# SciML/NeuralPDE.jl

Hardware: AMD Instinct MI355X
Metric: collocation-point residual+grad evals/sec, 2D Poisson 4x64 MLP (higher is better)
Workload: dtype f32, hidden-layer forward / dA / dW GEMMs as 3-piece bf16 split products (6 bf16 MFMAs per product block, fp32 accumulation; 24 mantissa bits rebuilt; the five small piece products on an accumulator of their own: zero-mean, a third of the rms error of an fp32-MFMA fmaf chain per GEMM output, tools/m

## Files before the change

### neuralpde.jl_amd/csrc/pinn_kernels2.hpp

```cpp
#pragma once
#include "pinn_kernels.hpp"

#if defined(PINN_STAMP) && !defined(PINN_EMU)
#define STAMP_MEMBERS unsigned st_acc[24]; unsigned long long st_last;
#define STAMP_INIT(ac) { for (int i_ = 0; i_ < 24; ++i_) (ac).st_acc[i_] = 0; (ac).st_last = __builtin_amdgcn_s_memtime(); }
#define STAMP(i) { const unsigned long long st_now = __builtin_amdgcn_s_memtime(); ac.st_acc[i] += (unsigned)(st_now - ac.st_last); ac.st_last = st_now; }
#define STAMP_EXTRA 128
#else
#define STAMP_MEMBERS
#define STAMP_INIT(ac)
#define STAMP(i)
#define STAMP_EXTRA 0
#endif

#ifndef PINN_F2_REC_LDS
#define PINN_F2_REC_LDS 1
#endif
#ifndef PINN_F2_SWP
#define PINN_F2_SWP 7
#endif
#ifndef PINN_PROBE
#define PINN_PROBE 0
#endif
#ifndef PINN_F2_ADJ_IL
#define PINN_F2_ADJ_IL 1
#endif
#ifndef PINN_F2_TR_FWDIMG
#define PINN_F2_TR_FWDIMG 1
#endif
#ifndef PINN_F2_SPLIT_ACC2
#define PINN_F2_SPLIT_ACC2 1
#endif
#ifndef PINN_F2_WACC_PRELOAD
#define PINN_F2_WACC_PRELOAD 2
#endif
#ifndef PINN_F2_MODES
#define PINN_F2_MODES 3
#endif

namespace pk {

constexpr int GEMM_FP32 = 0, GEMM_SPLIT = 1;
constexpr int F2_WAVES128 = 8;
constexpr int F2_NW8_MAXNG = 6;
constexpr int F2_GEMM_AHEAD = 2;
// ... 146 lines not shown
                ac.wLbar[t][r] = gload_masked(slab + S::O_WL, n, c0i);
            }
        if (w == 0) {
            const vbool l0 = veq(lane, 0);
            ac.bLbar = gload_masked(slab + S::O_BL, lane & vint(0), l0);
            PINN_UNROLL for (int j = 0; j < MAX_PARAMS; ++j) ac.pbar[j] = gload_masked(slab + S::O_P, vint(j) + (lane & vint(0)), l0);
        }
    }
}

template <class S, int MODE, int ACTK>
DEV void wave_tiles2(const GroupArgs& ga, int blk, int nblocks, int w, float* lds, Acc2<typename S::Shape>& ac,
                     int term_lo, int term_hi, int tile_lo, int tile_hi) {
    constexpr int HP = S::HP, MT = S::MT, MTW = S::MTW, NHH = S::NHH, LH = S::LH, D = S::D, C = S::C, PG = S::PG, NG = S::NG;
    constexpr int NFIRST = S::NFIRST;
    using J = typename S::J;
    constexpr bool BWD = (MODE == MODE_FUSED || MODE == MODE_GRADIN || MODE == MODE_GRADREC);
    constexpr bool SUMS = (MODE == MODE_FUSED || MODE == MODE_LOSS);
    constexpr bool TAPE_ONLY = (MODE == MODE_RESID || MODE == MODE_LOSS);
    constexpr bool RECOUT = (MODE == MODE_FWDREC), RECIN = (MODE == MODE_GRADREC);
    constexpr bool IS_FWD = (MODE == MODE_FWD || MODE == MODE_FWDREC), IS_GRADIN = (MODE == MODE_GRADIN || MODE == MODE_GRADREC);
    constexpr bool WPRE = (MT * MTW * 4 <= 16);
    constexpr bool TR_OVL = S::BFX_TR && WPRE && !S::CHUNKED;
    const int wave = blk * S::NW + w;
    const vint lane = lane_id();
    const vint g = lane >> 4;
    const vint c = lane & vint(15);
    const vbool g0 = veq(g, 0);
    const vint sw = S::BFX_TR ? (((g << 4) + (c ^ ((g >> 1) << 2))) << 1) : (lane << 2);
    vint trb[2];
    PINN_UNROLL for (int jh = 0; jh < 2; ++jh) {
        const vint gg = c & vint(3), pc = ((g & vint(1)) << 3) + vint(4 * jh) + (c >> 2);
        trb[jh] = (((gg << 4) + (pc ^ ((gg >> 1) << 2))) << 1);
    }
    vint trbq[2];
    PINN_UNROLL for (int jh = 0; jh < 2; ++jh) trbq[jh] = trb[jh] + (g >> 1) * vint(S::KB * 3 * 256);
    const vbool klo = vlt(g, 2);
    const float* P = ga.packed;
    constexpr int act = ACTK;
    static_assert(ACTK != ACT_MIXED, "per-layer activation kinds are compiled for family 1 (small nets) only");
    constexpr int ACLS = act_class(ACTK);
    constexpr bool RECZ = act_records_z(ACLS);
    const ubuf PB = ub_make(P, S::PACKED);
    const ubuf SB = ub_make(ga.scratch + (size_t)blk * (ga.scr_stride ? ga.scr_stride : S::SCR), S::SCR);
    float* X0 = lds;
    float* X1 = lds + S::OFF_X1;
// ... 6 lines not shown
    float* slab = ga.slabs + (size_t)blk * S::SLAB;
    auto& wbar = ac.wbar;
    auto& bbar = ac.bbar;
    auto& w1bar = ac.w1bar;
    auto& wLbar = ac.wLbar;
    vfloat& bLbar = ac.bLbar;
    auto& pbar = ac.pbar;
    vdacc& lsum = ac.lsum;
    int& cur_term = ac.cur_term;

    auto ld_wf = [&](int hl, int t, int mi) -> vfloat4 {
        return ub_load4(PB, S::OFF_WPK + ((hl * MT + w * MTW + t) * MT + mi) * 256, lane << 2);
    };
    auto ld_wt = [&](int hl, int t, int mo) -> vfloat4 {
        return ub_load4(PB, S::OFF_WTPK + ((hl * MT + w * MTW + t) * MT + mo) * 256, lane << 2);
    };
    auto ld_bias = [&](int layer, int t) -> vfloat4 { return ub_load4(PB, S::off_b(layer) + 16 * (w * MTW + t), g << 2); };

    vfloat4 wL[MTW];
    PINN_UNROLL for (int t = 0; t < MTW; ++t) wL[t] = ub_load4(PB, S::OFF_WL + 16 * (w * MTW + t), g << 2);
    const vbf8 wb_probe = ((PINN_PROBE & 8) && S::BFIMG) ? ub_load_bf8(PB, S::OFF_WB, lane << 2) : vbf8{};
    const float bL = P[S::OFF_BL];

    wave_prio(1);
    const int first = tile_lo + (((blk - tile_lo) % nblocks) + nblocks) % nblocks;
    for (int tix = first; tix < tile_hi; tix += nblocks) {
        STAMP(15)
        int k = term_lo;
        for (int j = term_lo + 1; j < term_hi; ++j)
            if (tix >= ga.terms[j].tile0) k = j;
        if (k != cur_term) {
            if (cur_term >= 0 && SUMS)
                ga.losspart[(size_t)wave * ga.nterms_total + ga.terms[cur_term].term_id] = wave_sum_dd(lsum, g0);
            lsum = vdacc_zero();
            cur_term = k;
        }
        const TermDev& T = ga.terms[k];
        const int pbase = (tix - T.tile0) * S::TP;
        const ubuf RB = ub_make((RECOUT || RECIN) ? ga.rec + (size_t)tix * S::REC : ga.scratch, S::REC);

        vfloat x[PG][D];
        vbool valid[PG];
        PINN_UNROLL for (int pg = 0; pg < PG; ++pg) {
            vint p = vint(pbase + 16 * pg) + c;
            valid[pg] = vlt(p, T.N);
            PINN_UNROLL for (int i = 0; i < D; ++i) x[pg][i] = gload_masked(T.pts, p * T.dt + vint(T.imap[i]), valid[pg]);
        }

        vfloat4 Rlast[NG][MTW];
        auto act_forward = [&](vfloat4 (&Z)[NG][MTW], int layer) {
            PINN_UNROLL for (int pg = 0; pg < PG; ++pg)
                PINN_UNROLL for (int t = 0; t < MTW; ++t) {
                    vfloat4 av;
                    av = act_value4<ACLS>(act, Z[pg * C][t]);
                    if (!RECZ) Z[pg * C][t] = av;
                    if (RECOUT && layer > 0)
                        PINN_UNROLL for (int ch = 0; ch < C; ++ch)
                            ub_store4(RB, (((layer - 1) * NG + pg * C + ch) * MT + w * MTW + t) * 256, lane << 2, Z[pg * C + ch][t]);
                    if (BWD) {
                        if (layer == LH - 1) {
                            PINN_UNROLL for (int ch = 0; ch < C; ++ch) Rlast[pg * C + ch][t] = Z[pg * C + ch][t];
                        } else if (layer > 0) {
                            PINN_UNROLL for (int ch = 0; ch < C; ++ch) {
                                if (rec_in_lds(layer, pg * C + ch)) lds_store4(RL, rl_off(layer, pg * C + ch, t), Z[pg * C + ch][t]);
                                else ub_store4(SB, (((layer - 1) * NG + pg * C + ch) * MT + w * MTW + t) * 256, lane << 2, Z[pg * C + ch][t]);
                            }
                        }
                    }
                    if ((RECOUT && layer > 0) || (BWD && layer > 0 && layer != LH - 1 && !rec_in_lds(layer, pg * C + C - 1))) {
// ... 110 lines not shown
                    PINN_UNROLL for (int sp = 0; sp < 3; ++sp) bb[(i + 1) % NB][sp] = ld_bfrag(X, (q2 * S::KB + kb2) * 3 + sp);
                }
                sched_fence();
                if (i + 1 < NGRP) lds_wait<3 * RD>(); else lds_wait<0>();
                PINN_UNROLL for (int t = 0; t < MTW; ++t) {
                    if (acc == 1) mfma_split2(wfr[kb][t], bb[i % NB], Cc[q][t], Cs[q][t]);
                    else Cc[q][t] = mfma_split(wfr[kb][t], bb[i % NB], Cc[q][t]);
                }
                chain_fence();
            }
            if (acc == 1)
                PINN_UNROLL for (int q = 0; q < NG; ++q)
                    PINN_UNROLL for (int t = 0; t < MTW; ++t)
                        PINN_UNROLL for (int e = 0; e < 4; ++e) Cc[q][t][e] += Cs[q][t][e];
        };
#ifndef PINN_F2_ACC_2PASS_ALL
#define PINN_F2_ACC_2PASS_ALL 0
#endif
        constexpr bool ACC_2PASS = PINN_F2_ACC_2PASS_ALL || (HP >= 128 && NG >= 5);
        auto acc_mode = [&](int bit) -> int { return (PINN_F2_SPLIT_ACC2 & bit) ? (ACC_2PASS ? 2 : 1) : 0; };

        vfloat4 A[NG][MTW];
        vfloat U[PG][C];
        constexpr int SRC_PRE = 2;
        vfloat srcv[SRC_PRE];
        PINN_UNROLL for (int j = 0; j < SRC_PRE; ++j) srcv[j] = vfloat(0.f);
        vbool valid_w = valid[0];
        PINN_UNROLL for (int pg = 1; pg < PG; ++pg) if (w == pg) valid_w = valid[pg];
        if (!RECIN) {
            PINN_UNROLL for (int t = 0; t < MTW; ++t) {
                const int n0 = 16 * (w * MTW + t);
                vfloat4 b1 = ub_load4(PB, S::off_b(0) + n0, g << 2);
                vfloat4 w1[D];
                PINN_UNROLL for (int i = 0; i < D; ++i) w1[i] = ub_load4(PB, S::OFF_W1 + i * HP + n0, g << 2);
                PINN_UNROLL for (int pg = 0; pg < PG; ++pg) {
                    vfloat4 z = b1;
                    PINN_UNROLL for (int i = 0; i < D; ++i)
                        PINN_UNROLL for (int r = 0; r < 4; ++r) z[r] = vfma(w1[i][r], x[pg][i], z[r]);
                    A[pg * C][t] = z;
                    PINN_UNROLL for (int kf = 0; kf < NFIRST; ++kf) A[pg * C + 1 + kf][t] = w1[S::first_axis(kf)];
                    PINN_UNROLL for (int ch = 1 + NFIRST; ch < C; ++ch) A[pg * C + ch][t] = vzero4();
                }
            }
            act_forward(A, 0);
            STAMP(0)
            PINN_UNROLL for (int hl = 0; hl < NHH; ++hl) {
                float* Xin = (hl & 1) ? X1 : X0;
// ... 52 lines not shown
                            PINN_UNROLL for (int t = 0; t < MTW; ++t)
                                PINN_UNROLL for (int e = 0; e < 4; ++e) A[q][t][e] += As[q][t][e];
                    if (WPRE && F2_GEMM_AHEAD > 0) sched_gemm_prefetch<S::KB * NG, MTW * 6, F2_GEMM_AHEAD, S::BFX_TR ? 6 : 3>();
                }
                PINN_UNROLL for (int mi = 0; mi < (S::BFX ? 0 : MT); ++mi) {
                    if (!WPRE)
                        PINN_UNROLL for (int t = 0; t < MTW; ++t)
                            wf[0][t] = ld_wf(hl, t, mi);
                    vfloat4 b4[NG];
                    PINN_UNROLL for (int q = 0; q < NG; ++q) b4[q] = lds_load4(Xin, vint(((q * MT + mi) * 64) * 4) + (lane << 2));
                    PINN_UNROLL for (int q = 0; q < NG; ++q)
                        PINN_UNROLL for (int t = 0; t < MTW; ++t)
                            PINN_UNROLL for (int rr = 0; rr < 4; ++rr) A[q][t] = mfma16(wf[WPRE ? mi : 0][t][rr], b4[q][rr], A[q][t]);
                }
                if (!S::BFX && WPRE && F2_GEMM_AHEAD > 0) sched_gemm_prefetch<MT * NG, MTW * 4, F2_GEMM_AHEAD>();
                wave_prio(1);
                STAMP(2)
                act_forward(A, hl + 1);
                STAMP(3)
            }
            if (MODE == MODE_FUSED || TAPE_ONLY)
                if (w < PG)
                    PINN_UNROLL for (int j = 0; j < SRC_PRE; ++j)
                        if (j < T.nsrc) srcv[j] = gload_masked(T.src, vint(j * T.N + pbase + 16 * w) + c, valid_w);
            {
                PINN_UNROLL for (int q = 0; q < NG; ++q) {
                    vfloat s = vfloat(0.f);
                    PINN_UNROLL for (int t = 0; t < MTW; ++t)
                        PINN_UNROLL for (int r = 0; r < 4; ++r) s = vfma(wL[t][r], A[q][t][r], s);
                    s = xrow_allsum(s);
                    lds_store(UP, vint((w * NG + q) * 16) + c, s);
                }
                wg_barrier();
            }
            PINN_UNROLL for (int pg = 0; pg < PG; ++pg)
                PINN_UNROLL for (int ch = 0; ch < C; ++ch) {
                    vfloat s = vfloat(0.f);
                    PINN_UNROLL for (int ws = 0; ws < S::NW; ++ws) s = s + lds_load(UP, vint((ws * NG + pg * C + ch) * 16) + c);
                    U[pg][ch] = (ch == 0) ? s + vfloat(bL) : s;
                }
        } else {
            PINN_UNROLL for (int pg = 0; pg < PG; ++pg)
                PINN_UNROLL for (int ch = 0; ch < C; ++ch) U[pg][ch] = vfloat(0.f);
            if (LH == 1) {
                PINN_UNROLL for (int t = 0; t < MTW; ++t) {
                    const int n0 = 16 * (w * MTW + t);
                    vfloat4 b1 = ub_load4(PB, S::off_b(0) + n0, g << 2);
// ... 11 lines not shown
                }
            } else {
                PINN_UNROLL for (int q = 0; q < NG; ++q)
                    PINN_UNROLL for (int t = 0; t < MTW; ++t)
                        Rlast[q][t] = ub_load4(RB, (((LH - 2) * NG + q) * MT + w * MTW + t) * 256, lane << 2);
            }
            PINN_UNROLL for (int pg = 0; pg < PG; ++pg)
                PINN_UNROLL for (int t = 0; t < MTW; ++t)
                    PINN_UNROLL for (int r = 0; r < 4; ++r) {
                        vfloat zz[C], dd[ND];
                        PINN_UNROLL for (int k2 = 0; k2 < C; ++k2) zz[k2] = Rlast[pg * C + k2][t][r];
                        act_derivs_n<J::NORD - 1, ACLS>(act, zz[0], dd);
                        jet_forward<J>(zz, dd);
                        A[pg * C][t][r] = act_from_record<ACLS>(Rlast[pg * C][t][r]);
                        PINN_UNROLL for (int k2 = 1; k2 < C; ++k2) A[pg * C + k2][t][r] = zz[k2];
                    }
        }
        STAMP(4)
        if (IS_FWD) {
            if (w == 0)
                PINN_UNROLL for (int pg = 0; pg < PG; ++pg) {
                    vint p = vint(pbase + 16 * pg) + c;
                    PINN_UNROLL for (int ch = 0; ch < C; ++ch)
                        gstore_masked(T.out, vint(ch * T.N) + p, U[pg][ch], vand(valid[pg], g0));
                }
            wg_barrier();
            continue;
        }

        constexpr bool SPRE = (NG * MTW * 4 <= F2_SPRE_MAX);
        vfloat4 Snext[SPRE ? NG : 1][SPRE ? MTW : 1];
        auto load_record = [&](int hl) {
            PINN_UNROLL for (int q = 0; q < NG; ++q)
                PINN_UNROLL for (int t = 0; t < MTW; ++t)
                    Snext[q][t] = (!RECIN && rec_in_lds(hl, q)) ? lds_load4(RL, rl_off(hl, q, t))
                                                             : ub_load4(RECIN ? RB : SB, (((hl - 1) * NG + q) * MT + w * MTW + t) * 256, lane << 2);
            sched_fence();
        };
        vfloat ubar[PG][C];
        if (IS_GRADIN) {
            PINN_UNROLL for (int pg = 0; pg < PG; ++pg) {
                vint p = vint(pbase + 16 * pg) + c;
                PINN_UNROLL for (int ch = 0; ch < C; ++ch) ubar[pg][ch] = gload_masked(T.in, vint(ch * T.N) + p, valid[pg]);
            }
            if (SPRE && NHH - 1 >= 1) load_record(NHH - 1);
        } else {
            float* UB = UP + S::NW * NG * 16;
            if (w < PG) {
                wave_prio(3);
                vfloat xin[D], Uin[C];
                vbool vin = valid[0];
                PINN_UNROLL for (int i = 0; i < D; ++i) xin[i] = x[0][i];
                PINN_UNROLL for (int ch = 0; ch < C; ++ch) Uin[ch] = U[0][ch];
                PINN_UNROLL for (int pg = 1; pg < PG; ++pg)
                    if (w == pg) {
                        vin = valid[pg];
                        PINN_UNROLL for (int i = 0; i < D; ++i) xin[i] = x[pg][i];
                        PINN_UNROLL for (int ch = 0; ch < C; ++ch) Uin[ch] = U[pg][ch];
                    }
                if (T.linear && C <= LIN_MAX_C) {
                    vfloat r = vfloat(T.lin_k);
                    PINN_UNROLL for (int ch = 0; ch < C; ++ch) r = vfma(vfloat(T.lin_a[ch < LIN_MAX_C ? ch : 0]), Uin[ch], r);
                    PINN_UNROLL for (int j = 0; j < LIN_MAX_SRC; ++j)
                        if (j < T.nsrc) {
                            vfloat sv;
                            if (j < SRC_PRE) { PINN_UNROLL for (int jj = 0; jj < SRC_PRE; ++jj) if (jj == j) sv = srcv[jj]; }
                            else sv = gload_masked(T.src, vint(j * T.N + pbase + 16 * w) + c, vin);
                            r = vfma(vfloat(T.lin_b[j]), sv, r);
                        }
                    if (MODE == MODE_RESID) {
                        vint p = vint(pbase + 16 * w) + c;
                        gstore_masked(T.out, p, r, vand(vin, g0));
                    } else {
                        vfloat sw = vfloat(1.0f);
                        if (T.pw) sw = gload_masked(T.pw, vint(pbase + 16 * w) + c, vin);
                        vfloat rm = vselect(vin, r * sw, vfloat(0.f));
                        lsum = vdacc_fma(rm, vselect(g0, rm, vfloat(0.f)), lsum);
                        if (MODE != MODE_LOSS) {
                            vfloat rbar = rm * vfloat(T.scale) * sw;
                            PINN_UNROLL for (int ch = 0; ch < C; ++ch)
                                lds_store(UB, vint((w * C + ch) * 16) + c, vselect(vin, rbar * vfloat(T.lin_a[ch < LIN_MAX_C ? ch : 0]), vfloat(0.f)));
                            if (T.src_bar)
                                PINN_UNROLL for (int j = 0; j < LIN_MAX_SRC; ++j)
                                    if (j < T.nsrc) gstore_masked(T.src_bar, vint(j * T.N + pbase + 16 * w) + c, rbar * vfloat(T.lin_b[j]), vand(vin, g0));
                        }
                    }
                } else {
                    const int NP = ga.nparams;
                    const int DT = T.dt;
                    const int R0 = DT + NP + C + T.nsrc;
                    const rp::Instr* prog = ga.prog + T.prog_off;
                    vtape tv;
                    tape_zero(tv);
                    if (!T.hetero) {
                        PINN_UNROLL for (int i = 0; i < D; ++i) tape_set(tv, i, xin[i]);
                    } else {
                        for (int j = 0; j < DT; ++j) tape_set(tv, j, gload_masked(T.pts, (vint(pbase + 16 * w) + c) * DT + vint(j), vin));
                    }
                    for (int j = 0; j < NP; ++j) tape_set(tv, DT + j, vfloat(ga.params[j]));
                    PINN_UNROLL for (int ch = 0; ch < C; ++ch) tape_set(tv, DT + NP + ch, Uin[ch]);
                    for (int j = 0; j < T.nsrc; ++j) {
                        vfloat sv;
                        if (j < SRC_PRE) { PINN_UNROLL for (int jj = 0; jj < SRC_PRE; ++jj) if (jj == j) sv = srcv[jj]; }
                        else sv = gload_masked(T.src, vint(j * T.N + pbase + 16 * w) + c, vin);
                        tape_set(tv, DT + NP + C + j, sv);
                    }
                    for (int q = 0; q < T.nops; ++q) {
                        const rp::Instr ins = rp::fetch_uniform(prog, q);
                        const vfloat va = tape_get(tv, ins.a), vb = tape_get(tv, ins.b);
                        vfloat vo;
                        if (rp::is_bilinear(ins.code)) vo = rp::apply_bilinear<vfloat>(ins, va, vb);
                        else vo = rp::apply<vfloat>(ins.code, va, vb, ins.imm);
                        tape_set(tv, R0 + q, vo);
                    }
                    vfloat r = tape_get(tv, T.out_row);
                    if (MODE == MODE_RESID) {
                        vint p = vint(pbase + 16 * w) + c;
                        gstore_masked(T.out, p, r, vand(vin, g0));
                    } else {
                        vfloat sw = vfloat(1.0f);
                        if (T.pw) sw = gload_masked(T.pw, vint(pbase + 16 * w) + c, vin);
                        vfloat rm = vselect(vin, r * sw, vfloat(0.f));
                        lsum = vdacc_fma(rm, vselect(g0, rm, vfloat(0.f)), lsum);
                        if (MODE != MODE_LOSS) {
                        vfloat rbar = rm * vfloat(T.scale) * sw;
                        vtape ta;
                        tape_zero(ta);
                        tape_set(ta, T.out_row, vfloat(1.0f));
                        for (int q = T.nops - 1; q >= 0; --q) {
                            const rp::Instr ins = rp::fetch_uniform(prog, q);
                            const vfloat va = tape_get(tv, ins.a), vb = tape_get(tv, ins.b), gq = tape_get(ta, R0 + q);
                            vfloat da, db;
                            if (rp::is_bilinear(ins.code)) rp::adjoint_bilinear<vfloat>(ins, va, vb, gq, da, db);
                            else rp::adjoint<vfloat>(ins.code, va, vb, tape_get(tv, R0 + q), ins.imm, gq, da, db);
                            tape_set(ta, ins.a, tape_get(ta, ins.a) + da);
                            tape_set(ta, ins.b, tape_get(ta, ins.b) + db);
                        }
                        PINN_UNROLL for (int ch = 0; ch < C; ++ch)
                            lds_store(UB, vint((w * C + ch) * 16) + c, vselect(vin, rbar * tape_get(ta, DT + NP + ch), vfloat(0.f)));
                        if (T.src_bar)
                            for (int j = 0; j < T.nsrc; ++j)
                                gstore_masked(T.src_bar, vint(j * T.N + pbase + 16 * w) + c, rbar * tape_get(ta, DT + NP + C + j), vand(vin, g0));
                        for (int j = 0; j < ga.nparams_estim; ++j) {
                            vfloat pj = vselect(vand(g0, vin), rbar * tape_get(ta, DT + j), vfloat(0.f));
                            PINN_UNROLL for (int jj = 0; jj < MAX_PARAMS; ++jj) if (jj == j) pbar[jj] += pj;
                        }
                        }
                    }
                }
                }
            wave_prio(1);
            if (!TAPE_ONLY) {
                if (SPRE && NHH - 1 >= 1) load_record(NHH - 1);
                wg_barrier();
                PINN_UNROLL for (int pg = 0; pg < PG; ++pg)
                    PINN_UNROLL for (int ch = 0; ch < C; ++ch) ubar[pg][ch] = lds_load(UB, vint((pg * C + ch) * 16) + c);
            }
        }
        if (TAPE_ONLY) { wg_barrier(); continue; }
        STAMP(5)

        constexpr bool FWD_IMG = S::BFX_TR && !RECIN && NHH >= 1 && PINN_F2_TR_FWDIMG;
        float* XA = (S::BFX_TR && ((NHH - 1) & 1) == 0) ? X0 : X1;
        float* XZ = (S::BFX_TR && ((NHH - 1) & 1) == 0) ? X1 : X0;
        auto ajet = [&](const vfloat4 (&Sr)[NG][MTW], int pg, int ch, int t) -> vfloat4 {
            vfloat4 out;
            PINN_UNROLL for (int r = 0; r < 4; ++r) {
                vfloat zz[C], dd[ND];
                PINN_UNROLL for (int k = 0; k < C; ++k) zz[k] = Sr[pg * C + k][t][r];
                if (ch > 0) {
                    act_derivs_n<J::NORD - 1, ACLS>(act, zz[0], dd);
                    jet_forward<J>(zz, dd);
                }
                out[r] = (ch == 0) ? act_from_record<ACLS>(zz[0]) : zz[ch];
            }
            return out;
        };
        auto act_adjoint = [&](vfloat4 (&G)[NG][MTW], const vfloat4 (&Sr)[NG][MTW]) {
            PINN_UNROLL for (int pg = 0; pg < PG; ++pg)
                PINN_UNROLL for (int t = 0; t < MTW; ++t)
                    PINN_UNROLL for (int r = 0; r < 4; ++r) {
                        vfloat gg[C], ss[C], dd[ND];
// ... 170 lines not shown
            };
            vfloat4 wt[WPRE ? MT : 1][MTW];
            vbf8 wtb[S::BFX ? S::KB : 1][S::BFX ? MTW : 1][3];
            if (S::BFX) {
                PINN_UNROLL for (int kb = 0; kb < S::KB; ++kb)
                    PINN_UNROLL for (int t = 0; t < MTW; ++t)
                        PINN_UNROLL for (int sp = 0; sp < 3; ++sp)
                            wtb[kb][t][sp] = (PINN_PROBE & 8) ? wb_probe : ub_load_bf8(PB, S::OFF_WTB + (((hl * MT + w * MTW + t) * S::KB + kb) * 3 + sp) * 256, lane << 2);
                sched_fence();
            } else if (WPRE) {
                PINN_UNROLL for (int mo = 0; mo < MT; ++mo)
                    PINN_UNROLL for (int t = 0; t < MTW; ++t)
                        wt[mo][t] = ld_wt(hl, t, mo);
                sched_fence();
            }
            vfloat4 Gn[NG][MTW];
            PINN_UNROLL for (int q = 0; q < NG; ++q)
                PINN_UNROLL for (int t = 0; t < MTW; ++t) Gn[q][t] = vzero4();
            constexpr bool OVL = WPRE && !S::CHUNKED;
            if (OVL) {
                STAMP(7)
                wg_barrier();
                STAMP(8)
                if (SPRE && hl - 1 >= 1) load_record(hl - 1);
                wave_prio(0);
                if (S::BFX_TR && (PINN_F2_SWP & 2)) gemm_swp(XZ, wtb, Gn, acc_mode(2));
                PINN_UNROLL for (int q = 0; q < ((S::BFX_TR && (PINN_F2_SWP & 2)) ? 0 : NG); ++q) {
                    if (S::BFX) {
                        constexpr bool ACC2 = (PINN_F2_SPLIT_ACC2 & 2) != 0;
                        vfloat4 Gs[MTW];
                        PINN_UNROLL for (int t = 0; t < MTW; ++t) Gs[t] = vzero4();
                        PINN_UNROLL for (int kb = 0; kb < S::KB; ++kb) {
                            vbf8 bb[3];
                            PINN_UNROLL for (int sp = 0; sp < 3; ++sp) bb[sp] = ld_bfrag(XZ, (q * S::KB + kb) * 3 + sp);
                            PINN_UNROLL for (int t = 0; t < MTW; ++t) {
                                if (ACC2) mfma_split2(wtb[kb][t], bb, Gn[q][t], Gs[t]);
                                else Gn[q][t] = mfma_split(wtb[kb][t], bb, Gn[q][t]);
                            }
                        }
                        if (ACC2)
                            PINN_UNROLL for (int t = 0; t < MTW; ++t)
                                PINN_UNROLL for (int e = 0; e < 4; ++e) Gn[q][t][e] += Gs[t][e];
                    } else {
                        PINN_UNROLL for (int mo = 0; mo < MT; ++mo) {
                            vfloat4 b4 = lds_load4(X0, vint(((q * MT + mo) * 64) * 4) + (lane << 2));
                            PINN_UNROLL for (int t = 0; t < MTW; ++t)
// ... 125 lines not shown
            }
            STAMP(10)
            wg_barrier();
            STAMP(11)
            if (!ADJ_IL) {
                PINN_UNROLL for (int q = 0; q < NG; ++q)
                    PINN_UNROLL for (int t = 0; t < MTW; ++t) G[q][t] = Gn[q][t];
                act_adjoint(G, Sr);
            }
            STAMP(12)
        }
        PINN_UNROLL for (int pg = 0; pg < PG; ++pg)
            PINN_UNROLL for (int t = 0; t < MTW; ++t)
                PINN_UNROLL for (int r = 0; r < 4; ++r) {
                    const vfloat gz = G[pg * C][t][r];
                    bbar[0][t][r] += gz;
                    PINN_UNROLL for (int i = 0; i < D; ++i) w1bar[i][t][r] = vfma(gz, x[pg][i], w1bar[i][t][r]);
                    PINN_UNROLL for (int kf = 0; kf < NFIRST; ++kf)
                        PINN_UNROLL for (int i = 0; i < D; ++i)
                            if (i == S::first_axis(kf)) w1bar[i][t][r] += G[pg * C + 1 + kf][t][r];
                }
        if (NHH == 0) wg_barrier();
        STAMP(13)
    }
}

template <class S, int PG = S::PG >
DEV void acc2_store(Acc2<typename S::Shape>& ac, const GroupArgs& ga, int blk, int w, float* lds) {
    constexpr int HP = S::HP, MT = S::MT, MTW = S::MTW, NHH = S::NHH, LH = S::LH, D = S::D, NG = S::NG;
    const vint lane = lane_id();
    const vint g = lane >> 4;
    const vint c = lane & vint(15);
    float* slab = ga.slabs + (size_t)blk * S::SLAB;
    float* UP = lds + S::OFF_UP;
    if (S::WBAR_REG)
        PINN_UNROLL for (int hl = 0; hl < NHH; ++hl)
            PINN_UNROLL for (int t = 0; t < MTW; ++t)
                PINN_UNROLL for (int ti = 0; ti < MT; ++ti)
                    gstore4(slab + S::O_WBAR, vint((((hl * MT + w * MTW + t) * MT + ti) * 64) * 4) + (lane << 2), ac.wbar[hl][t][ti]);
    const vbool c0 = veq(c, 0);
    auto reduce_cols = [&](vfloat v) -> vfloat {
        v = row_allsum16(v);
        return v;
    };
    PINN_UNROLL for (int t = 0; t < MTW; ++t)
        PINN_UNROLL for (int r = 0; r < 4; ++r) {
// ... 12 lines not shown
    if (w == 0) {
        float s = (float)wave_sum_d(ac.bLbar, all);
        gstore_masked(slab + S::O_BL, vint(0), vfloat(s), veq(lane, 0));
        PINN_UNROLL for (int j = 0; j < MAX_PARAMS; ++j) {
            vfloat sp = vfloat((float)wave_sum_d(ac.pbar[j], all));
            PINN_UNROLL for (int ws = 1; ws < PG; ++ws) sp = sp + lds_load(UBp, vint(ws * MAX_PARAMS + j) + (lane & vint(0)));
            gstore_masked(slab + S::O_P, vint(j), sp, veq(lane, 0));
        }
    }
#if defined(PINN_STAMP) && !defined(PINN_EMU)
    STAMP(14)
    if ((threadIdx.x & 63) == 0)
        for (int i = 0; i < 24; ++i) reinterpret_cast<unsigned*>(slab + S::SLAB - 128)[w * 24 + i] = ac.st_acc[i];
#endif
}

template <class S, int MODE, int ACTK>
DEV void wave_main2(const GroupArgs& ga, int blk, int nblocks, int w, float* lds) {
    constexpr bool BWD = (MODE == MODE_FUSED || MODE == MODE_GRADIN || MODE == MODE_GRADREC);
    constexpr bool SUMS = (MODE == MODE_FUSED || MODE == MODE_LOSS);
    const int wave = blk * S::NW + w;
    Acc2<typename S::Shape> ac;
    acc2_init<S>(ac, ga, blk, w, BWD);
    if (SUMS)
        for (int j = 0; j < ga.nterms; ++j) ga.losspart[(size_t)wave * ga.nterms_total + ga.terms[j].term_id] = 0.0;
    wave_tiles2<S, MODE, ACTK>(ga, blk, nblocks, w, lds, ac, 0, ga.nterms, 0, ga.ntiles);
    if (SUMS && ac.cur_term >= 0)
        ga.losspart[(size_t)wave * ga.nterms_total + ga.terms[ac.cur_term].term_id] = wave_sum_dd(ac.lsum, veq(lane_id() >> 4, 0));
    if (!BWD) return;
    acc2_store<S>(ac, ga, blk, w, lds);
}

template <class S0, class S1, int ACTK, int MODE = MODE_FUSED>
DEV void wave_main2m(const GroupArgs& ga, int blk, int nblocks, int w, float* lds) {
    static_assert(same_type<typename S0::Shape, typename S1::Shape>::value, "merged launches need members of one network shape and neuron split");
    static_assert(S0::SLAB == S1::SLAB && S0::PACKED == S1::PACKED, "merged launches share the slab and the packed weight image");
    static_assert(S0::DW_NATURAL == S1::DW_NATURAL && S0::BFX_TR == S1::BFX_TR, "merged launches: one order of the dW tiles in the slab, one exchange-image layout");
    static_assert(MODE == MODE_FUSED || MODE == MODE_LOSS, "merged launches: the fused evaluation and the loss-only evaluation");
    const int wave = blk * S0::NW + w;
    Acc2<typename S0::Shape> ac;
    acc2_init<S0>(ac, ga, blk, w, MODE == MODE_FUSED);
    for (int j = 0; j < ga.nterms; ++j) ga.losspart[(size_t)wave * ga.nterms_total + ga.terms[j].term_id] = 0.0;
    wave_tiles2<S0, MODE, ACTK>(ga, blk, nblocks, w, lds, ac, 0, ga.sub_terms0, 0, ga.sub_tiles0);
    wg_barrier();
    wave_tiles2<S1, MODE, ACTK>(ga, blk, nblocks, w, lds, ac, ga.sub_terms0, ga.nterms, ga.sub_tiles0, ga.ntiles);
    if (ac.cur_term >= 0)
        ga.losspart[(size_t)wave * ga.nterms_total + ga.terms[ac.cur_term].term_id] = wave_sum_dd(ac.lsum, veq(lane_id() >> 4, 0));
    if (MODE != MODE_FUSED) return;
    wg_barrier();
    acc2_store<S0, (S0::PG > S1::PG ? S0::PG : S1::PG)>(ac, ga, blk, w, lds);
}

}
```

### neuralpde.jl_amd/csrc/vec.hpp

```cpp
#pragma once
#ifndef __HIPCC_RTC__
#include <cmath>
#include <cstdint>
#include <cstring>
#include <type_traits>
#endif

#ifdef PINN_EMU
#define DEV inline
#define HD inline
#define PINN_UNROLL
namespace wv {
constexpr int W = 64;
struct vbool { bool v[W]; };
struct vint {
    int v[W];
    vint() {}
    vint(int s) { for (int l = 0; l < W; ++l) v[l] = s; }
};
struct vfloat {
    float v[W];
    vfloat() {}
    vfloat(float s) { for (int l = 0; l < W; ++l) v[l] = s; }
};
// ... 54 lines not shown
#undef VFN1
inline vfloat vpow(const vfloat& a, const vfloat& b) { vfloat r; for (int l = 0; l < W; ++l) r.v[l] = std::pow(a.v[l], b.v[l]); return r; }
inline vfloat vmax(const vfloat& a, const vfloat& b) { vfloat r; for (int l = 0; l < W; ++l) r.v[l] = a.v[l] > b.v[l] ? a.v[l] : b.v[l]; return r; }
inline vfloat vmin(const vfloat& a, const vfloat& b) { vfloat r; for (int l = 0; l < W; ++l) r.v[l] = a.v[l] < b.v[l] ? a.v[l] : b.v[l]; return r; }
inline vbool vlt(const vint& a, int b) { vbool r; for (int l = 0; l < W; ++l) r.v[l] = a.v[l] < b; return r; }
inline vbool veq(const vint& a, int b) { vbool r; for (int l = 0; l < W; ++l) r.v[l] = a.v[l] == b; return r; }
inline vbool vgt(const vfloat& a, const vfloat& b) { vbool r; for (int l = 0; l < W; ++l) r.v[l] = a.v[l] > b.v[l]; return r; }
inline vbool vand(const vbool& a, const vbool& b) { vbool r; for (int l = 0; l < W; ++l) r.v[l] = a.v[l] && b.v[l]; return r; }
inline vfloat vselect(const vbool& m, const vfloat& a, const vfloat& b) { vfloat r; for (int l = 0; l < W; ++l) r.v[l] = m.v[l] ? a.v[l] : b.v[l]; return r; }
inline vint vselect(const vbool& m, const vint& a, const vint& b) { vint r; for (int l = 0; l < W; ++l) r.v[l] = m.v[l] ? a.v[l] : b.v[l]; return r; }
inline vfloat gload(const float* p, const vint& i) { vfloat r; for (int l = 0; l < W; ++l) r.v[l] = p[i.v[l]]; return r; }
inline vfloat gload_masked(const float* p, const vint& i, const vbool& m) { vfloat r; for (int l = 0; l < W; ++l) r.v[l] = m.v[l] ? p[i.v[l]] : 0.f; return r; }
inline void gstore(float* p, const vint& i, const vfloat& x) { for (int l = 0; l < W; ++l) p[i.v[l]] = x.v[l]; }
inline void gstore_masked(float* p, const vint& i, const vfloat& x, const vbool& m) { for (int l = 0; l < W; ++l) if (m.v[l]) p[i.v[l]] = x.v[l]; }
inline vfloat4 gload4(const float* p, const vint& i) { vfloat4 r; for (int k = 0; k < 4; ++k) for (int l = 0; l < W; ++l) r.x[k].v[l] = p[i.v[l] + k]; return r; }
inline void gstore4(float* p, const vint& i, const vfloat4& x) { for (int k = 0; k < 4; ++k) for (int l = 0; l < W; ++l) p[i.v[l] + k] = x.x[k].v[l]; }
struct vtape { vfloat r[32]; };
inline vfloat tape_get(const vtape& t, int i) { return t.r[i]; }
inline void tape_set(vtape& t, int i, const vfloat& x) { t.r[i] = x; }
inline void tape_zero(vtape& t) { for (int i = 0; i < 32; ++i) t.r[i] = vfloat(0.f); }
struct urec16 { int x, y, z, w; };
inline void sched_fence() {}
inline int opaque_lane(int x) { return x; }
template <int N> inline void lds_wait() {}
inline void chain_fence() {}
inline void store_pad() {}
inline void keep_alive(const vfloat4&) {}
inline void wave_prio(int) {}
template <int NGROUPS, int MFMA_PER, int AHEAD, int DS_PER = 1> inline void sched_gemm_prefetch() {}
inline void vsincos(const vfloat& x, vfloat& s, vfloat& c) { for (int l = 0; l < W; ++l) { s.v[l] = std::sin(x.v[l]); c.v[l] = std::cos(x.v[l]); } }
inline urec16 uload16(const void* p) { urec16 r; std::memcpy(&r, p, 16); return r; }
struct urec32 { int v[8]; };
inline urec32 uload32(const void* p) { urec32 r; std::memcpy(&r, p, 32); return r; }
struct ubuf { float* p; };
inline ubuf ub_make(const float* p, size_t) { return ubuf{const_cast<float*>(p)}; }
inline vfloat4 ub_load4(const ubuf& b, int soff, const vint& voff) { vfloat4 r; for (int k = 0; k < 4; ++k) for (int l = 0; l < W; ++l) r.x[k].v[l] = b.p[soff + voff.v[l] + k]; return r; }
inline vfloat4 ub_load4_sc1(const ubuf& b, int soff, const vint& voff) { return ub_load4(b, soff, voff); }
inline void ub_store4(const ubuf& b, int soff, const vint& voff, const vfloat4& x) { for (int k = 0; k < 4; ++k) for (int l = 0; l < W; ++l) b.p[soff + voff.v[l] + k] = x.x[k].v[l]; }
inline vfloat ub_load(const ubuf& b, int soff, const vint& voff) { vfloat r; for (int l = 0; l < W; ++l) r.v[l] = b.p[soff + voff.v[l]]; return r; }
inline vfloat ub_load_sc1(const ubuf& b, int soff, const vint& voff) { return ub_load(b, soff, voff); }
inline void ub_store4_wt(const ubuf& b, const vint& voff, const vfloat4& x) { for (int k = 0; k < 4; ++k) for (int l = 0; l < W; ++l) b.p[voff.v[l] + k] = x.x[k].v[l]; }
inline void gstore_masked_wt(float* p, const vint& i, const vfloat& x, const vbool& m) { for (int l = 0; l < W; ++l) if (m.v[l]) p[i.v[l]] = x.v[l]; }
inline void ustore_wt(double* p, double x) { *p = x; }
inline void ustore_wt(float* p, float x) { *p = x; }
inline float uload_wt(const float* p) { return *p; }
inline double uload_wt(const double* p) { return *p; }
// ... 294 lines not shown
DEV ubuf ub_make(const float* p, size_t nfloats) {
    return ubuf{__builtin_amdgcn_make_buffer_rsrc(const_cast<float*>(p), 0, (int)(nfloats * 4), 0x00020000)};
}
DEV vfloat4 ub_load4(ubuf b, int soff, vint voff) {
    return __builtin_bit_cast(vfloat4, __builtin_amdgcn_raw_buffer_load_b128(b.r, voff * 4, soff * 4, 0));
}
DEV vfloat4 ub_load4_sc1(ubuf b, int soff, vint voff) {
    return __builtin_bit_cast(vfloat4, __builtin_amdgcn_raw_buffer_load_b128(b.r, voff * 4, soff * 4, 16));
}
DEV void ub_store4(ubuf b, int soff, vint voff, vfloat4 x) {
    __builtin_amdgcn_raw_buffer_store_b128(__builtin_bit_cast(vuint4, x), b.r, voff * 4, soff * 4, 0);
}
DEV vfloat ub_load(ubuf b, int soff, vint voff) {
    return __builtin_bit_cast(float, __builtin_amdgcn_raw_buffer_load_b32(b.r, voff * 4, soff * 4, 0));
}
template <int AUX> DEV double ub_loadd(ubuf b, int soff, vint voff) {
    return __builtin_bit_cast(double, __builtin_amdgcn_raw_buffer_load_b64(b.r, voff * 8, soff * 8, AUX));
}
template <int AUX> DEV float ub_loadf(ubuf b, int soff, vint voff) {
    return __builtin_bit_cast(float, __builtin_amdgcn_raw_buffer_load_b32(b.r, voff * 4, soff * 4, AUX));
}
DEV void opaque_v(int& x) { asm volatile("" : "+v"(x)); }
DEV void opaque_s(int& x) { asm volatile("" : "+s"(x)); }
DEV vfloat ub_load_sc1(ubuf b, int soff, vint voff) {
    return __builtin_bit_cast(float, __builtin_amdgcn_raw_buffer_load_b32(b.r, voff * 4, soff * 4, 16));
}
DEV void ub_store4_wt(ubuf b, vint voff, vfloat4 x) {
    __builtin_amdgcn_raw_buffer_store_b128(__builtin_bit_cast(vuint4, x), b.r, voff * 4, 0, 16);
}
DEV void gstore_masked_wt(float* p, vint i, vfloat x, vbool m) { if (m) __hip_atomic_store(p + i, x, __ATOMIC_RELAXED, __HIP_MEMORY_SCOPE_AGENT); }
DEV void ustore_wt(double* p, double x) { __hip_atomic_store(p, x, __ATOMIC_RELAXED, __HIP_MEMORY_SCOPE_AGENT); }
DEV void ustore_wt(float* p, float x) { __hip_atomic_store(p, x, __ATOMIC_RELAXED, __HIP_MEMORY_SCOPE_AGENT); }
DEV float uload_wt(const float* p) { return __hip_atomic_load(p, __ATOMIC_RELAXED, __HIP_MEMORY_SCOPE_AGENT); }
DEV double uload_wt(const double* p) { return __hip_atomic_load(p, __ATOMIC_RELAXED, __HIP_MEMORY_SCOPE_AGENT); }
DEV vfloat lds_load(const float* p, vint i) { return p[i]; }
DEV void lds_store(float* p, vint i, vfloat x) { p[i] = x; }
DEV vfloat4 lds_load4(const float* p, vint i) { return *reinterpret_cast<const vfloat4*>(p + i); }
DEV void lds_store4(float* p, vint i, vfloat4 x) { *reinterpret_cast<vfloat4*>(p + i) = x; }
DEV void wave_fence() {
    __builtin_amdgcn_fence(__ATOMIC_RELEASE, "wavefront");
    __builtin_amdgcn_wave_barrier();
    __builtin_amdgcn_fence(__ATOMIC_ACQUIRE, "wavefront");
}
#ifndef PINN_PROBE
#define PINN_PROBE 0
#endif
// ... 197 lines not shown
```

Baseline: 231.6 million.

## Prefetch next tile's collocation points and cache term fields in scalar registers

Moves the per-tile point loads into a tile_head routine that runs for the next tile during the current tile's work: after the first hidden-layer barrier, or at the end of the tile. This hides global-load latency behind the GEMMs. Term descriptor fields are copied once per term change into a struct pinned to SGPRs, so the tile loop no longer re-reads them from memory, and the term lookup becomes an incremental advance. The losspart zeroing loop is replaced by a lane-parallel store. The cost is extra registers to hold the prefetched points, plus possible register-pressure or scheduling changes from the pinning asm.

After: 233.8 million (median of 6 runs). About the same (+0.9%).

```diff
diff --git a/neuralpde.jl_amd/csrc/pinn_kernels2.hpp b/neuralpde.jl_amd/csrc/pinn_kernels2.hpp
--- a/neuralpde.jl_amd/csrc/pinn_kernels2.hpp
+++ b/neuralpde.jl_amd/csrc/pinn_kernels2.hpp
@@ -21,6 +21,18 @@
 #endif
 #ifndef PINN_PROBE
 #define PINN_PROBE 0
+#endif
+#ifndef PINN_F2_XPRE
+#define PINN_F2_XPRE 2
+#endif
+#ifndef PINN_F2_XPRE_PGMAX
+#define PINN_F2_XPRE_PGMAX 1
+#endif
+#ifndef PINN_F2_TPIN
+#define PINN_F2_TPIN 1
+#endif
+#ifndef PINN_F2_WOPQ
+#define PINN_F2_WOPQ 1
 #endif
 #ifndef PINN_F2_ADJ_IL
 #define PINN_F2_ADJ_IL 1
@@ -213,6 +225,7 @@
     constexpr bool IS_FWD = (MODE == MODE_FWD || MODE == MODE_FWDREC), IS_GRADIN = (MODE == MODE_GRADIN || MODE == MODE_GRADREC);
     constexpr bool WPRE = (MT * MTW * 4 <= 16);
     constexpr bool TR_OVL = S::BFX_TR && WPRE && !S::CHUNKED;
+    constexpr bool OVL_LAST = BWD && WPRE && !S::CHUNKED && NHH >= 1;
     const int wave = blk * S::NW + w;
     const vint lane = lane_id();
     const vint g = lane >> 4;
@@ -265,29 +278,64 @@
     const vbf8 wb_probe = ((PINN_PROBE & 8) && S::BFIMG) ? ub_load_bf8(PB, S::OFF_WB, lane << 2) : vbf8{};
     const float bL = P[S::OFF_BL];
 
-    wave_prio(1);
-    const int first = tile_lo + (((blk - tile_lo) % nblocks) + nblocks) % nblocks;
-    for (int tix = first; tix < tile_hi; tix += nblocks) {
-        STAMP(15)
-        int k = term_lo;
-        for (int j = term_lo + 1; j < term_hi; ++j)
-            if (tix >= ga.terms[j].tile0) k = j;
-        if (k != cur_term) {
+    constexpr int XPRE = (PG <= PINN_F2_XPRE_PGMAX) ? PINN_F2_XPRE : 0;
+    constexpr int SRC_PRE = 2;
+    constexpr int CL = (C <= LIN_MAX_C) ? C : 1;
+    struct TermS {
+        const float* pts; const float* src;
+        int N, tile0, dt, nsrc, imap[D];
+        int linear, has_pw, has_src_bar;
+        int scale, lin_k, lin_a[CL], lin_b[SRC_PRE];
+    } ts;
+    int kterm = term_lo;
+    int next_tile0 = (term_lo + 1 < term_hi) ? ga.terms[term_lo + 1].tile0 : 0x7fffffff;
+    vfloat xn[PG][D];
+    auto tile_head = [&](int tix) {
+        while (tix >= next_tile0) {
+            ++kterm;
+            next_tile0 = (kterm + 1 < term_hi) ? ga.terms[kterm + 1].tile0 : 0x7fffffff;
+        }
+        if (kterm != cur_term) {
             if (cur_term >= 0 && SUMS)
                 ga.losspart[(size_t)wave * ga.nterms_total + ga.terms[cur_term].term_id] = wave_sum_dd(lsum, g0);
             lsum = vdacc_zero();
-            cur_term = k;
+            cur_term = kterm;
+            const TermDev& Tn = ga.terms[kterm];
+            ts.pts = Tn.pts; ts.src = Tn.src; ts.N = Tn.N; ts.tile0 = Tn.tile0; ts.dt = Tn.dt; ts.nsrc = Tn.nsrc;
+            ts.linear = Tn.linear; ts.has_pw = ptr_bits_or(Tn.pw); ts.has_src_bar = ptr_bits_or(Tn.src_bar);
+            ts.scale = sbits(Tn.scale); ts.lin_k = sbits(Tn.lin_k);
+            if (PINN_F2_TPIN) { pin_s(ts.pts); pin_s(ts.src); pin_s(ts.N); pin_s(ts.tile0); pin_s(ts.dt); pin_s(ts.nsrc);
+            pin_s(ts.linear); pin_s(ts.has_pw); pin_s(ts.has_src_bar); pin_s(ts.scale); pin_s(ts.lin_k); }
+            PINN_UNROLL for (int i = 0; i < D; ++i) { ts.imap[i] = Tn.imap[i]; if (PINN_F2_TPIN) pin_s(ts.imap[i]); }
+            PINN_UNROLL for (int ch = 0; ch < CL; ++ch) { ts.lin_a[ch] = sbits(Tn.lin_a[ch]); if (PINN_F2_TPIN) pin_s(ts.lin_a[ch]); }
+            PINN_UNROLL for (int j = 0; j < SRC_PRE; ++j) { ts.lin_b[j] = sbits(Tn.lin_b[j]); if (PINN_F2_TPIN) pin_s(ts.lin_b[j]); }
+            if (PINN_F2_TPIN) { pin_s(kterm); pin_s(next_tile0); }
         }
-        const TermDev& T = ga.terms[k];
-        const int pbase = (tix - T.tile0) * S::TP;
+        const int pb = (tix - ts.tile0) * S::TP;
+        PINN_UNROLL for (int pg = 0; pg < PG; ++pg) {
+            const vint p = vint(pb + 16 * pg) + c;
+            const vbool v = vlt(p, ts.N);
+            PINN_UNROLL for (int i = 0; i < D; ++i) xn[pg][i] = gload_masked(ts.pts, p * ts.dt + vint(ts.imap[i]), v);
+        }
+    };
+
+    wave_prio(1);
+    const int first = tile_lo + (((blk - tile_lo) % nblocks) + nblocks) % nblocks;
+    if (XPRE && first < tile_hi) tile_head(first);
+    for (int tix = first; tix < tile_hi; tix += nblocks) {
+        STAMP(15)
+        if (PINN_F2_WOPQ) pin_s(w);
+        if (!XPRE) tile_head(tix);
+        auto next_head = [&]() { if (XPRE && tix + nblocks < tile_hi) tile_head(tix + nblocks); };
+        const TermDev& T = ga.terms[kterm];
+        const int pbase = (tix - ts.tile0) * S::TP;
         const ubuf RB = ub_make((RECOUT || RECIN) ? ga.rec + (size_t)tix * S::REC : ga.scratch, S::REC);
 
         vfloat x[PG][D];
         vbool valid[PG];
         PINN_UNROLL for (int pg = 0; pg < PG; ++pg) {
-            vint p = vint(pbase + 16 * pg) + c;
-            valid[pg] = vlt(p, T.N);
-            PINN_UNROLL for (int i = 0; i < D; ++i) x[pg][i] = gload_masked(T.pts, p * T.dt + vint(T.imap[i]), valid[pg]);
+            valid[pg] = vlt(vint(pbase + 16 * pg) + c, ts.N);
+            PINN_UNROLL for (int i = 0; i < D; ++i) x[pg][i] = xn[pg][i];
         }
 
         vfloat4 Rlast[NG][MTW];
@@ -444,7 +492,6 @@
 
         vfloat4 A[NG][MTW];
         vfloat U[PG][C];
-        constexpr int SRC_PRE = 2;
         vfloat srcv[SRC_PRE];
         PINN_UNROLL for (int j = 0; j < SRC_PRE; ++j) srcv[j] = vfloat(0.f);
         vbool valid_w = valid[0];
@@ -543,7 +590,7 @@
             if (MODE == MODE_FUSED || TAPE_ONLY)
                 if (w < PG)
                     PINN_UNROLL for (int j = 0; j < SRC_PRE; ++j)
-                        if (j < T.nsrc) srcv[j] = gload_masked(T.src, vint(j * T.N + pbase + 16 * w) + c, valid_w);
+                        if (j < ts.nsrc) srcv[j] = gload_masked(ts.src, vint(j * ts.N + pbase + 16 * w) + c, valid_w);
             {
                 PINN_UNROLL for (int q = 0; q < NG; ++q) {
                     vfloat s = vfloat(0.f);
@@ -601,9 +648,10 @@
                 PINN_UNROLL for (int pg = 0; pg < PG; ++pg) {
                     vint p = vint(pbase + 16 * pg) + c;
                     PINN_UNROLL for (int ch = 0; ch < C; ++ch)
-                        gstore_masked(T.out, vint(ch * T.N) + p, U[pg][ch], vand(valid[pg], g0));
+                        gstore_masked(T.out, vint(ch * ts.N) + p, U[pg][ch], vand(valid[pg], g0));
                 }
             wg_barrier();
+            next_head();
             continue;
         }
 
@@ -620,7 +668,7 @@
         if (IS_GRADIN) {
             PINN_UNROLL for (int pg = 0; pg < PG; ++pg) {
                 vint p = vint(pbase + 16 * pg) + c;
-                PINN_UNROLL for (int ch = 0; ch < C; ++ch) ubar[pg][ch] = gload_masked(T.in, vint(ch * T.N) + p, valid[pg]);
+                PINN_UNROLL for (int ch = 0; ch < C; ++ch) ubar[pg][ch] = gload_masked(T.in, vint(ch * ts.N) + p, valid[pg]);
             }
             if (SPRE && NHH - 1 >= 1) load_record(NHH - 1);
         } else {
@@ -637,51 +685,51 @@
                         PINN_UNROLL for (int i = 0; i < D; ++i) xin[i] = x[pg][i];
                         PINN_UNROLL for (int ch = 0; ch < C; ++ch) Uin[ch] = U[pg][ch];
                     }
-                if (T.linear && C <= LIN_MAX_C) {
-                    vfloat r = vfloat(T.lin_k);
-                    PINN_UNROLL for (int ch = 0; ch < C; ++ch) r = vfma(vfloat(T.lin_a[ch < LIN_MAX_C ? ch : 0]), Uin[ch], r);
+                if (ts.linear && C <= LIN_MAX_C) {
+                    vfloat r = vfloat(sfloat(ts.lin_k));
+                    PINN_UNROLL for (int ch = 0; ch < C; ++ch) r = vfma(vfloat(sfloat(ts.lin_a[ch < CL ? ch : 0])), Uin[ch], r);
                     PINN_UNROLL for (int j = 0; j < LIN_MAX_SRC; ++j)
-                        if (j < T.nsrc) {
+                        if (j < ts.nsrc) {
                             vfloat sv;
                             if (j < SRC_PRE) { PINN_UNROLL for (int jj = 0; jj < SRC_PRE; ++jj) if (jj == j) sv = srcv[jj]; }
-                            else sv = gload_masked(T.src, vint(j * T.N + pbase + 16 * w) + c, vin);
-                            r = vfma(vfloat(T.lin_b[j]), sv, r);
+                            else sv = gload_masked(ts.src, vint(j * ts.N + pbase + 16 * w) + c, vin);
+                            r = vfma(vfloat(j < SRC_PRE ? sfloat(ts.lin_b[j < SRC_PRE ? j : 0]) : T.lin_b[j]), sv, r);
                         }
                     if (MODE == MODE_RESID) {
                         vint p = vint(pbase + 16 * w) + c;
                         gstore_masked(T.out, p, r, vand(vin, g0));
                     } else {
                         vfloat sw = vfloat(1.0f);
-                        if (T.pw) sw = gload_masked(T.pw, vint(pbase + 16 * w) + c, vin);
+                        if (ts.has_pw) sw = gload_masked(T.pw, vint(pbase + 16 * w) + c, vin);
                         vfloat rm = vselect(vin, r * sw, vfloat(0.f));
                         lsum = vdacc_fma(rm, vselect(g0, rm, vfloat(0.f)), lsum);
                         if (MODE != MODE_LOSS) {
-                            vfloat rbar = rm * vfloat(T.scale) * sw;
+                            vfloat rbar = rm * vfloat(sfloat(ts.scale)) * sw;
                             PINN_UNROLL for (int ch = 0; ch < C; ++ch)
-                                lds_store(UB, vint((w * C + ch) * 16) + c, vselect(vin, rbar * vfloat(T.lin_a[ch < LIN_MAX_C ? ch : 0]), vfloat(0.f)));
-                            if (T.src_bar)
+                                lds_store(UB, vint((w * C + ch) * 16) + c, vselect(vin, rbar * vfloat(sfloat(ts.lin_a[ch < CL ? ch : 0])), vfloat(0.f)));
+                            if (ts.has_src_bar)
                                 PINN_UNROLL for (int j = 0; j < LIN_MAX_SRC; ++j)
-                                    if (j < T.nsrc) gstore_masked(T.src_bar, vint(j * T.N + pbase + 16 * w) + c, rbar * vfloat(T.lin_b[j]), vand(vin, g0));
+                                    if (j < ts.nsrc) gstore_masked(T.src_bar, vint(j * ts.N + pbase + 16 * w) + c, rbar * vfloat(T.lin_b[j]), vand(vin, g0));
                         }
                     }
                 } else {
                     const int NP = ga.nparams;
-                    const int DT = T.dt;
-                    const int R0 = DT + NP + C + T.nsrc;
+                    const int DT = ts.dt;
+                    const int R0 = DT + NP + C + ts.nsrc;
                     const rp::Instr* prog = ga.prog + T.prog_off;
                     vtape tv;
                     tape_zero(tv);
                     if (!T.hetero) {
                         PINN_UNROLL for (int i = 0; i < D; ++i) tape_set(tv, i, xin[i]);
                     } else {
-                        for (int j = 0; j < DT; ++j) tape_set(tv, j, gload_masked(T.pts, (vint(pbase + 16 * w) + c) * DT + vint(j), vin));
+                        for (int j = 0; j < DT; ++j) tape_set(tv, j, gload_masked(ts.pts, (vint(pbase + 16 * w) + c) * DT + vint(j), vin));
                     }
                     for (int j = 0; j < NP; ++j) tape_set(tv, DT + j, vfloat(ga.params[j]));
                     PINN_UNROLL for (int ch = 0; ch < C; ++ch) tape_set(tv, DT + NP + ch, Uin[ch]);
-                    for (int j = 0; j < T.nsrc; ++j) {
+                    for (int j = 0; j < ts.nsrc; ++j) {
                         vfloat sv;
                         if (j < SRC_PRE) { PINN_UNROLL for (int jj = 0; jj < SRC_PRE; ++jj) if (jj == j) sv = srcv[jj]; }
-                        else sv = gload_masked(T.src, vint(j * T.N + pbase + 16 * w) + c, vin);
+                        else sv = gload_masked(ts.src, vint(j * ts.N + pbase + 16 * w) + c, vin);
                         tape_set(tv, DT + NP + C + j, sv);
                     }
                     for (int q = 0; q < T.nops; ++q) {
@@ -698,11 +746,11 @@
                         gstore_masked(T.out, p, r, vand(vin, g0));
                     } else {
                         vfloat sw = vfloat(1.0f);
-                        if (T.pw) sw = gload_masked(T.pw, vint(pbase + 16 * w) + c, vin);
+                        if (ts.has_pw) sw = gload_masked(T.pw, vint(pbase + 16 * w) + c, vin);
                         vfloat rm = vselect(vin, r * sw, vfloat(0.f));
                         lsum = vdacc_fma(rm, vselect(g0, rm, vfloat(0.f)), lsum);
                         if (MODE != MODE_LOSS) {
-                        vfloat rbar = rm * vfloat(T.scale) * sw;
+                        vfloat rbar = rm * vfloat(sfloat(ts.scale)) * sw;
                         vtape ta;
                         tape_zero(ta);
                         tape_set(ta, T.out_row, vfloat(1.0f));
@@ -717,9 +765,9 @@
                         }
                         PINN_UNROLL for (int ch = 0; ch < C; ++ch)
                             lds_store(UB, vint((w * C + ch) * 16) + c, vselect(vin, rbar * tape_get(ta, DT + NP + ch), vfloat(0.f)));
-                        if (T.src_bar)
-                            for (int j = 0; j < T.nsrc; ++j)
-                                gstore_masked(T.src_bar, vint(j * T.N + pbase + 16 * w) + c, rbar * tape_get(ta, DT + NP + C + j), vand(vin, g0));
+                        if (ts.has_src_bar)
+                            for (int j = 0; j < ts.nsrc; ++j)
+                                gstore_masked(T.src_bar, vint(j * ts.N + pbase + 16 * w) + c, rbar * tape_get(ta, DT + NP + C + j), vand(vin, g0));
                         for (int j = 0; j < ga.nparams_estim; ++j) {
                             vfloat pj = vselect(vand(g0, vin), rbar * tape_get(ta, DT + j), vfloat(0.f));
                             PINN_UNROLL for (int jj = 0; jj < MAX_PARAMS; ++jj) if (jj == j) pbar[jj] += pj;
@@ -736,7 +784,7 @@
                     PINN_UNROLL for (int ch = 0; ch < C; ++ch) ubar[pg][ch] = lds_load(UB, vint((pg * C + ch) * 16) + c);
             }
         }
-        if (TAPE_ONLY) { wg_barrier(); continue; }
+        if (TAPE_ONLY) { wg_barrier(); next_head(); continue; }
         STAMP(5)
 
         constexpr bool FWD_IMG = S::BFX_TR && !RECIN && NHH >= 1 && PINN_F2_TR_FWDIMG;
@@ -953,6 +1001,7 @@
                 STAMP(7)
                 wg_barrier();
                 STAMP(8)
+                if (XPRE >= 2 && hl == 0) next_head();
                 if (SPRE && hl - 1 >= 1) load_record(hl - 1);
                 wave_prio(0);
                 if (S::BFX_TR && (PINN_F2_SWP & 2)) gemm_swp(XZ, wtb, Gn, acc_mode(2));
@@ -1124,6 +1173,7 @@
                 }
         if (NHH == 0) wg_barrier();
         STAMP(13)
+        if (!(XPRE >= 2 && OVL_LAST)) next_head();
     }
 }
 
@@ -1182,8 +1232,7 @@
     const int wave = blk * S::NW + w;
     Acc2<typename S::Shape> ac;
     acc2_init<S>(ac, ga, blk, w, BWD);
-    if (SUMS)
-        for (int j = 0; j < ga.nterms; ++j) ga.losspart[(size_t)wave * ga.nterms_total + ga.terms[j].term_id] = 0.0;
+    if (SUMS) gzero_d_indexed(ga.losspart + (size_t)wave * ga.nterms_total, &ga.terms[0].term_id, (int)(sizeof(TermDev) / sizeof(int)), ga.nterms);
     wave_tiles2<S, MODE, ACTK>(ga, blk, nblocks, w, lds, ac, 0, ga.nterms, 0, ga.ntiles);
     if (SUMS && ac.cur_term >= 0)
         ga.losspart[(size_t)wave * ga.nterms_total + ga.terms[ac.cur_term].term_id] = wave_sum_dd(ac.lsum, veq(lane_id() >> 4, 0));
@@ -1200,7 +1249,7 @@
     const int wave = blk * S0::NW + w;
     Acc2<typename S0::Shape> ac;
     acc2_init<S0>(ac, ga, blk, w, MODE == MODE_FUSED);
-    for (int j = 0; j < ga.nterms; ++j) ga.losspart[(size_t)wave * ga.nterms_total + ga.terms[j].term_id] = 0.0;
+    gzero_d_indexed(ga.losspart + (size_t)wave * ga.nterms_total, &ga.terms[0].term_id, (int)(sizeof(TermDev) / sizeof(int)), ga.nterms);
     wave_tiles2<S0, MODE, ACTK>(ga, blk, nblocks, w, lds, ac, 0, ga.sub_terms0, 0, ga.sub_tiles0);
     wg_barrier();
     wave_tiles2<S1, MODE, ACTK>(ga, blk, nblocks, w, lds, ac, ga.sub_terms0, ga.nterms, ga.sub_tiles0, ga.ntiles);
diff --git a/neuralpde.jl_amd/csrc/vec.hpp b/neuralpde.jl_amd/csrc/vec.hpp
--- a/neuralpde.jl_amd/csrc/vec.hpp
+++ b/neuralpde.jl_amd/csrc/vec.hpp
@@ -100,6 +100,11 @@
 struct urec16 { int x, y, z, w; };
 inline void sched_fence() {}
 inline int opaque_lane(int x) { return x; }
+template <class T> inline void pin_s(T&) {}
+inline int sbits(float x) { int r; std::memcpy(&r, &x, 4); return r; }
+inline float sfloat(int b) { float r; std::memcpy(&r, &b, 4); return r; }
+inline int ptr_bits_or(const void* p) { const unsigned long long a = (unsigned long long)p; return (int)((unsigned)a | (unsigned)(a >> 32)); }
+inline void gzero_d_indexed(double* base, const int* idx, int stride, int n) { for (int j = 0; j < n; ++j) base[idx[j * stride]] = 0.0; }
 template <int N> inline void lds_wait() {}
 inline void chain_fence() {}
 inline void store_pad() {}
@@ -440,6 +445,14 @@
 }
 DEV void opaque_v(int& x) { asm volatile("" : "+v"(x)); }
 DEV void opaque_s(int& x) { asm volatile("" : "+s"(x)); }
+template <class T> DEV void pin_s(T& x) { asm volatile("" : "+s"(x)); }
+DEV int sbits(float x) { return __builtin_bit_cast(int, x); }
+DEV float sfloat(int b) { return __builtin_bit_cast(float, b); }
+DEV int ptr_bits_or(const void* p) { const unsigned long long a = (unsigned long long)p; return (int)((unsigned)a | (unsigned)(a >> 32)); }
+DEV void gzero_d_indexed(double* base, const int* idx, int stride, int n) {
+    const int j = (int)(threadIdx.x & 63);
+    if (j < n) base[idx[j * stride]] = 0.0;
+}
 DEV vfloat ub_load_sc1(ubuf b, int soff, vint voff) {
     return __builtin_bit_cast(float, __builtin_amdgcn_raw_buffer_load_b32(b.r, voff * 4, soff * 4, 16));
 }
```
